# QwenLM/Qwen3-TTS

Hardware: NVIDIA B200
Metric: speech_tokens_per_s (higher is better)
Workload: dtype bf16

## Files before the change

qwen3-tts_b200/csrc/ar_sampler.cuh:

```cuda
#pragma once

namespace {

__device__ __forceinline__ unsigned int fkey(float f) {
  unsigned int u = __float_as_uint(f);
  return (u & 0x80000000u) ? ~u : (u | 0x80000000u);
}

__device__ __noinline__ float kth_largest(const float* sv, int V, int k, unsigned int* hist, int* sh) {
  unsigned int prefix = 0, mask = 0;
#pragma unroll 1
  for (int pass = 3; pass >= 0; --pass) {
    const int shift = pass * 8;
    if (threadIdx.x < 256) hist[threadIdx.x] = 0;
    cta_sync();
#pragma unroll 1
    for (int i = threadIdx.x; i < V; i += NTHREADS) {
      const unsigned int key = fkey(sv[i]);
      if ((key & mask) == prefix) atomicAdd(&hist[(key >> shift) & 255u], 1u);
    }
    cta_sync();
    unsigned int cnt = 0, incl = 0;
    if (threadIdx.x < 256) {
      cnt = hist[threadIdx.x];
      incl = cnt;
      const int ln = threadIdx.x & 31;
#pragma unroll
      for (int o = 1; o < 32; o <<= 1) {
        unsigned int n = __shfl_down_sync(0xffffffffu, incl, o);
        if (ln + o < 32) incl += n;
      }
      if (ln == 0) sh[threadIdx.x >> 5] = (int)incl;
    }
    cta_sync();
    if (threadIdx.x < 256) {
      unsigned int above = 0;
#pragma unroll 1
      for (int w = (threadIdx.x >> 5) + 1; w < 8; ++w) above += (unsigned int)sh[w];
      incl += above;
      const unsigned int excl = incl - cnt;
      if ((int)excl < k && k <= (int)incl) { sh[8] = threadIdx.x; sh[9] = k - (int)excl; }
    }
    cta_sync();
    prefix |= ((unsigned int)sh[8]) << shift;
    mask |= 255u << shift;
    k = sh[9];
    cta_sync();
  }
  const unsigned int u = (prefix & 0x80000000u) ? (prefix & 0x7fffffffu) : ~prefix;
  return __uint_as_float(u);
}

__device__ __noinline__ bool sample_fast(const float* sv, int V, int k, float u, float* scratch, float* red, int* ired, int* tok_out) {
  int* hist = reinterpret_cast<int*>(scratch);
  float* cand = scratch + 2048;
  int* kidx = reinterpret_cast<int*>(scratch + 2048 + 256);
  float* kp = scratch + 2048 + 256 + 384;
  int* sidx = reinterpret_cast<int*>(scratch + 2048 + 256 + 768);
  float* spp = scratch + 2048 + 256 + 1152;
  __shared__ int s_misc[8];
  const int tid = threadIdx.x, lane = tid & 31, wp = tid >> 5;
  float mx = -INFINITY;
#pragma unroll 1
  for (int i = tid; i < V; i += NTHREADS) mx = fmaxf(mx, sv[i]);
  mx = block_reduce(mx, red, 0);
#pragma unroll 1
  for (int i = tid; i < 2048; i += NTHREADS) hist[i] = 0;
  if (tid == 0) { s_misc[0] = -1; s_misc[2] = 0; s_misc[3] = 0; s_misc[4] = __float_as_int(-INFINITY); }
  cta_sync();
  const float lo = mx - 32.f;
#pragma unroll 1
  for (int i = tid; i < V; i += NTHREADS) {
    const float sc = sv[i];
    if (sc > -INFINITY) atomicAdd(&hist[min(2047, max(0, (int)((sc - lo) * 64.f)))], 1);
  }
  cta_sync();
  int hb[8], S = 0;
#pragma unroll
  for (int j = 0; j < 8; ++j) { hb[j] = hist[8 * tid + j]; S += hb[j]; }
  int incl = S;
#pragma unroll
  for (int o = 1; o < 32; o <<= 1) {
    const int n = __shfl_down_sync(0xffffffffu, incl, o);
    if (lane + o < 32) incl += n;
  }
  if (lane == 0) ired[wp] = incl;
  cta_sync();
  int above = incl - S;
#pragma unroll 1
  for (int w = wp + 1; w < NWARPS; ++w) above += ired[w];
  {
    int run = above;
#pragma unroll
    for (int j = 7; j >= 0; --j) {
      if (run < k && k <= run + hb[j]) { s_misc[0] = 8 * tid + j; s_misc[1] = k - run; }
      run += hb[j];
    }
  }
  cta_sync();
  const int tb = s_misc[0], kk = s_misc[1];
  if (tb < 0) return false;
#pragma unroll 1
  for (int i = tid; i < V; i += NTHREADS) {
    const float sc = sv[i];
    if (sc > -INFINITY && min(2047, max(0, (int)((sc - lo) * 64.f))) == tb) {
      const int p = atomicAdd(&s_misc[2], 1);
      if (p < 256) cand[p] = sc;
    }
  }
  cta_sync();
  const int nc = s_misc[2];
  if (nc > 256) return false;
  if (tid < nc) {
    const float v = cand[tid];
    int gt = 0, ge = 0;
#pragma unroll 1
    for (int j = 0; j < nc; ++j) { const float w = cand[j]; gt += w > v; ge += w >= v; }
    if (gt < kk && kk <= ge) s_misc[4] = __float_as_int(v);
  }
  cta_sync();
  const float thr = __int_as_float(s_misc[4]);
#pragma unroll 1
  for (int i = tid; i < V; i += NTHREADS) {
    const float sc = sv[i];
    if (sc > -INFINITY && sc >= thr) {
      const int p = atomicAdd(&s_misc[3], 1);
      if (p < 384) { kidx[p] = i; kp[p] = __expf(sc - mx); }
    }
  }
  cta_sync();
  const int m = s_misc[3];
  if (m > 384 || m == 0) return false;
#pragma unroll 1
  for (int e = tid; e < m; e += NTHREADS) {
    const int id = kidx[e];
    int r = 0;
#pragma unroll 1
    for (int j = 0; j < m; ++j) r += kidx[j] < id;
    sidx[r] = id;
    spp[r] = kp[e];
  }
  cta_sync();
  if (tid < 32) {
    const int per = (m + 31) >> 5;
    const int a = min(m, lane * per), bnd = min(m, a + per);
    float loc = 0.f;
#pragma unroll 1
    for (int j = a; j < bnd; ++j) loc += spp[j];
    float inc = loc;
#pragma unroll
    for (int o = 1; o < 32; o <<= 1) {
      const float n = __shfl_up_sync(0xffffffffu, inc, o);
      if (lane >= o) inc += n;
    }
    const float total = __shfl_sync(0xffffffffu, inc, 31);
    const float target = u * total;
    float run = inc - loc;
    int cnd = 0x7fffffff;
#pragma unroll 1
    for (int j = a; j < bnd; ++j) {
      run += spp[j];
      if (run > target && cnd == 0x7fffffff && spp[j] > 0.f) cnd = j;
    }
#pragma unroll
    for (int o = 16; o > 0; o >>= 1) cnd = min(cnd, __shfl_xor_sync(0xffffffffu, cnd, o));
    if (cnd == 0x7fffffff) {
      int last = -1;
#pragma unroll 1
      for (int j = a; j < bnd; ++j)
        if (spp[j] > 0.f) last = j;
#pragma unroll
      for (int o = 16; o > 0; o >>= 1) last = max(last, __shfl_xor_sync(0xffffffffu, last, o));
      cnd = max(last, 0);
    }
    if (lane == 0) s_misc[5] = sidx[cnd];
  }
  cta_sync();
  *tok_out = s_misc[5];
  return true;
}

__device__ __forceinline__ void sample_phase(const Phase& ph, const KParams& P, unsigned char* smem, int frame, bool in_prefill) {
  const int b = blockIdx.x;
  DevState* st = P.st;
  const int B = P.B;
  if (b >= B) return;
  if (in_prefill && !((P.admit_mask >> b) & 1u)) return;
  frame -= P.frame0[b];
  const int tid = threadIdx.x;
  const int group = ph.group;
  const bool talker = group == 0;
  const StackDev& S = talker ? P.talker : P.cp;
  const int V = S.vocab;
  const int H = P.talker.hidden;
  float* sv = reinterpret_cast<float*>(smem);
  float* pv = sv + MAXV;
  float* red = pv + MAXV;
  int* ired = reinterpret_cast<int*>(red + 32);
  unsigned int* hist = reinterpret_cast<unsigned int*>(ired + 32);
  const int fidx = talker ? (in_prefill ? 0 : frame + 1) : frame;
  const bool do_sample = talker ? P.sp.do_sample : P.sp.subtalker_dosample;
  const float temperature = talker ? P.sp.temperature : P.sp.subtalker_temperature;
  const int top_k = talker ? P.sp.top_k : P.sp.subtalker_top_k;
  const float top_p = talker ? P.sp.top_p : P.sp.subtalker_top_p;
  const float* lg = S.logits + (size_t)b * V;
  const int n_gen_b = talker ? ldcgi(&st->n_gen[b]) : 0;

  {
    float lreg[MAXV / NTHREADS];
#pragma unroll
    for (int r = 0; r < MAXV / NTHREADS; ++r) { const int i = tid + r * NTHREADS; if (i < V) lreg[r] = ldcgf(lg + i); }
#pragma unroll
    for (int r = 0; r < MAXV / NTHREADS; ++r) { const int i = tid + r * NTHREADS; if (i < V) sv[i] = lreg[r]; }
  }
  float* dbg = talker ? (P.dbg_tlogits ? P.dbg_tlogits + ((size_t)fidx * B + b) * V : nullptr)
                      : (P.dbg_clogits ? P.dbg_clogits + (((size_t)frame * (P.G - 1) + (group - 1)) * B + b) * V : nullptr);
  const float rp = P.sp.repetition_penalty;
  const float inv_t = (do_sample && temperature != 1.0f) ? temperature : 1.0f;
#pragma unroll 1
  for (int i = tid; i < V; i += NTHREADS) {
    float s = sv[i];
    if (dbg) dbg[i] = s;
    if (talker) {
      if (rp != 1.0f && __ldcg(P.seen + (size_t)b * V + i)) s = s < 0.f ? s * rp : s / rp;
      if (i == P.eos && (n_gen_b < P.sp.min_new_tokens || P.sp.suppress_eos)) s = -INFINITY;
      if (i >= V - 1024 && i != P.eos) s = -INFINITY;
    }
    if (inv_t != 1.0f) s = s / inv_t;
    sv[i] = s;
  }
  cta_sync();

  int tok;
  if (!do_sample) {
    float mx = -INFINITY;
#pragma unroll 1
    for (int i = tid; i < V; i += NTHREADS) mx = fmaxf(mx, sv[i]);
    mx = block_reduce(mx, red, 0);
    int idx = 0x7fffffff;
#pragma unroll 1
    for (int i = tid; i < V; i += NTHREADS)
      if (sv[i] == mx) idx = min(idx, i);
    tok = block_min_int(idx, ired);
  } else if (top_p >= 1.0f && top_k > 0 && top_k < V && top_k <= 128 &&
             sample_fast(sv, V, top_k, philox_uniform(P.sp.seed, P.row_key[b], (uint32_t)fidx, (uint32_t)group), pv, red, ired, &tok)) {
  } else {
    if (top_k > 0 && top_k < V) {
      const float thr = kth_largest(sv, V, top_k, hist, ired);
#pragma unroll 1
      for (int i = tid; i < V; i += NTHREADS)
        if (sv[i] < thr) sv[i] = -INFINITY;
      cta_sync();
    }
    float mx = -INFINITY;
#pragma unroll 1
    for (int i = tid; i < V; i += NTHREADS) mx = fmaxf(mx, sv[i]);
    mx = block_reduce(mx, red, 0);
    if (top_p < 1.0f) {
      float tot = 0.f;
#pragma unroll 1
      for (int i = tid; i < V; i += NTHREADS) { const float p = __expf(sv[i] - mx); pv[i] = p; tot += p; }
      tot = block_reduce(tot, red, 1);
      cta_sync();
      unsigned int rm_mask = 0;
      int slot = 0;
#pragma unroll 1
      for (int i = tid; i < V; i += NTHREADS, ++slot) {
        const float si = sv[i];
        bool rm = false;
        if (si != -INFINITY) {
          float cum = 0.f;
          bool is_top = true;
#pragma unroll 1
          for (int j = 0; j < V; ++j) {
            const float sj = sv[j];
            if (sj == -INFINITY) continue;
            if (sj < si || (sj == si && j <= i)) cum += pv[j];
            if (sj > si || (sj == si && j > i)) is_top = false;
          }
          rm = (cum / tot <= 1.0f - top_p) && !is_top;
        }
        if (rm) rm_mask |= 1u << slot;
      }
      cta_sync();
      slot = 0;
#pragma unroll 1
      for (int i = tid; i < V; i += NTHREADS, ++slot)
        if (rm_mask & (1u << slot)) sv[i] = -INFINITY;
      cta_sync();
    }
    const int E = (V + NTHREADS - 1) / NTHREADS;
    const int i0 = tid * E, i1 = min(V, i0 + E);
    float loc = 0.f;
#pragma unroll 1
    for (int i = i0; i < i1; ++i) { const float p = __expf(sv[i] - mx); pv[i] = p; loc += p; }
    float incl = loc;
    const int ln = tid & 31, wp = tid >> 5;
#pragma unroll
    for (int o = 1; o < 32; o <<= 1) {
      const float n = __shfl_up_sync(0xffffffffu, incl, o);
      if (ln >= o) incl += n;
    }
    cta_sync();
    if (ln == 31) red[wp] = incl;
    cta_sync();
    float base = 0.f, total = 0.f;
#pragma unroll 1
    for (int w = 0; w < NWARPS; ++w) { if (w < wp) base += red[w]; total += red[w]; }
    const float excl = base + incl - loc;
    const float u = philox_uniform(P.sp.seed, P.row_key[b], (uint32_t)fidx, (uint32_t)group);
    const float target = u * total;
    int cand = 0x7fffffff, lastpos = -1;
    float run = excl;
#pragma unroll 1
    for (int i = i0; i < i1; ++i) {
      run += pv[i];
      if (pv[i] > 0.f) { lastpos = i; if (run > target && cand == 0x7fffffff) cand = i; }
    }
    cand = block_min_int(cand, ired);
    if (cand == 0x7fffffff) cand = -block_min_int(-lastpos, ired);
    tok = cand;
  }
  if (P.forced && fidx < P.n_forced) {
    const int f = P.forced[((size_t)b * P.n_forced + fidx) * P.G + group];
    if (f >= 0) tok = f;
  }

  if (talker) {
    const int was_finished = ldcgi(&st->finished[b]);
    if (was_finished) tok = P.eos;
    cta_sync();
    if (tid == 0) {
      if (!was_finished) {
        if (tok == P.eos) { st->finished[b] = 1; st->n_valid[b] = fidx; }
        else { P.seen[(size_t)b * V + tok] = 1; }
        st->n_gen[b] = n_gen_b + 1;
      }
      st->c0[b] = tok;
      st->cur[b][0] = tok;
    }
    bf16* x1 = P.x_cp + ((size_t)B + b) * H;
    bf16* x0 = P.x_cp + (size_t)b * H;
    const bf16* e = P.emb_t + (size_t)tok * H;
    const bf16* ph_ = P.past_hidden + (size_t)b * H;
#pragma unroll 1
    for (int i = tid * 8; i < H; i += NTHREADS * 8) {
      *reinterpret_cast<uint4*>(x1 + i) = *reinterpret_cast<const uint4*>(e + i);
      *reinterpret_cast<uint4*>(x0 + i) = ldcg16(ph_ + i);
    }
  } else {
    const int j = group;
    if (tid == 0) {
      st->cur[b][j] = tok;
      if (P.codes_out && frame >= 0 && frame < P.codes_stride) {
        int* row = P.codes_out + ((size_t)b * P.codes_stride + frame) * P.G;
        row[j] = tok;
        if (j == 1) row[0] = ldcgi(&st->cur[b][0]);
      }
    }
    cta_sync();
    const int Vc = P.cp.vocab;
    if (j < P.G - 1) {
      const int Wn = P.cp_next_w;
      const bf16* e = P.cp_next + ((size_t)(j - 1) * Vc + tok) * Wn;
      bf16* x = P.cp_next_dst + (size_t)b * Wn;
#pragma unroll 1
      for (int i = tid * 8; i < Wn; i += NTHREADS * 8)
        *reinterpret_cast<uint4*>(x + i) = *reinterpret_cast<const uint4*>(e + i);
    } else {
      const bf16* txt = (frame < P.trailing_len[b])
                            ? P.trailing + ((size_t)b * P.trailing_stride + frame) * H
                            : P.tts_pad;
      int* codes = reinterpret_cast<int*>(hist);
      if (tid < P.G) codes[tid] = (tid == j) ? tok : ldcgi(&st->cur[b][tid]);
      cta_sync();
#pragma unroll 1
      for (int i = tid; i < H; i += NTHREADS) {
        float s = bf2f(P.emb_t[(size_t)codes[0] * H + i]);
#pragma unroll 4
        for (int g2 = 1; g2 < P.G; ++g2) s += bf2f(P.emb_cp[((size_t)(g2 - 1) * Vc + codes[g2]) * H + i]);
        P.talker.h[(size_t)b * H + i] = f2bf(rbf(s) + bf2f(txt[i]));
      }
    }
  }
}

}
```

Before: 2070.

## Fuse max into preprocessing and drop extra vocab pass in fast top-k sampler

The running max is now computed inside the penalty/temperature loop, which removes a separate pass over the vocabulary in both the greedy and sampling paths. The histogram is zeroed during preprocessing, so one barrier disappears. In the fast top-k sampler, the candidate-collection pass also gathers every token above the threshold bin, and candidates inside the threshold bin are selected directly by rank. This removes the final full-vocabulary threshold scan. The trade-off is extra shared scratch for candidate indices and a different ordering in kidx, which the later rank-sort handles.

```diff
diff --git a/qwen3-tts_b200/csrc/ar_sampler.cuh b/qwen3-tts_b200/csrc/ar_sampler.cuh
--- a/qwen3-tts_b200/csrc/ar_sampler.cuh
+++ b/qwen3-tts_b200/csrc/ar_sampler.cuh
@@ -51,23 +51,20 @@
   return __uint_as_float(u);
 }
 
-__device__ __noinline__ bool sample_fast(const float* sv, int V, int k, float u, float* scratch, float* red, int* ired, int* tok_out) {
+__device__ __noinline__ bool sample_fast(const float* sv, int V, int k, float u, float* scratch, float* red, int* ired, int* tok_out,
+                                         float mx_part) {
   int* hist = reinterpret_cast<int*>(scratch);
   float* cand = scratch + 2048;
-  int* kidx = reinterpret_cast<int*>(scratch + 2048 + 256);
-  float* kp = scratch + 2048 + 256 + 384;
-  int* sidx = reinterpret_cast<int*>(scratch + 2048 + 256 + 768);
-  float* spp = scratch + 2048 + 256 + 1152;
+  int* cidx = reinterpret_cast<int*>(scratch + 2048 + 256);
+  int* kidx = reinterpret_cast<int*>(scratch + 2048 + 512);
+  float* kp = scratch + 2048 + 512 + 384;
+  int* sidx = reinterpret_cast<int*>(scratch + 2048 + 512 + 768);
+  float* spp = scratch + 2048 + 512 + 1152;
+  static_assert(2048 + 512 + 1536 <= MAXV, "sampler scratch");
   __shared__ int s_misc[8];
   const int tid = threadIdx.x, lane = tid & 31, wp = tid >> 5;
-  float mx = -INFINITY;
-#pragma unroll 1
-  for (int i = tid; i < V; i += NTHREADS) mx = fmaxf(mx, sv[i]);
-  mx = block_reduce(mx, red, 0);
-#pragma unroll 1
-  for (int i = tid; i < 2048; i += NTHREADS) hist[i] = 0;
-  if (tid == 0) { s_misc[0] = -1; s_misc[2] = 0; s_misc[3] = 0; s_misc[4] = __float_as_int(-INFINITY); }
-  cta_sync();
+  if (tid == 0) { s_misc[0] = -1; s_misc[2] = 0; s_misc[3] = 0; }
+  const float mx = block_reduce(mx_part, red, 0);
   const float lo = mx - 32.f;
 #pragma unroll 1
   for (int i = tid; i < V; i += NTHREADS) {
@@ -103,9 +100,15 @@
 #pragma unroll 1
   for (int i = tid; i < V; i += NTHREADS) {
     const float sc = sv[i];
-    if (sc > -INFINITY && min(2047, max(0, (int)((sc - lo) * 64.f))) == tb) {
-      const int p = atomicAdd(&s_misc[2], 1);
-      if (p < 256) cand[p] = sc;
+    if (sc > -INFINITY) {
+      const int bin = min(2047, max(0, (int)((sc - lo) * 64.f)));
+      if (bin == tb) {
+        const int p = atomicAdd(&s_misc[2], 1);
+        if (p < 256) { cand[p] = sc; cidx[p] = i; }
+      } else if (bin > tb) {
+        const int p = atomicAdd(&s_misc[3], 1);
+        if (p < 384) { kidx[p] = i; kp[p] = __expf(sc - mx); }
+      }
     }
   }
   cta_sync();
@@ -113,19 +116,12 @@
   if (nc > 256) return false;
   if (tid < nc) {
     const float v = cand[tid];
-    int gt = 0, ge = 0;
-#pragma unroll 1
-    for (int j = 0; j < nc; ++j) { const float w = cand[j]; gt += w > v; ge += w >= v; }
-    if (gt < kk && kk <= ge) s_misc[4] = __float_as_int(v);
-  }
-  cta_sync();
-  const float thr = __int_as_float(s_misc[4]);
-#pragma unroll 1
-  for (int i = tid; i < V; i += NTHREADS) {
-    const float sc = sv[i];
-    if (sc > -INFINITY && sc >= thr) {
+    int gt = 0;
+#pragma unroll 1
+    for (int j = 0; j < nc; ++j) gt += cand[j] > v;
+    if (gt < kk) {
       const int p = atomicAdd(&s_misc[3], 1);
-      if (p < 384) { kidx[p] = i; kp[p] = __expf(sc - mx); }
+      if (p < 384) { kidx[p] = cidx[tid]; kp[p] = __expf(v - mx); }
     }
   }
   cta_sync();
@@ -217,6 +213,13 @@
                       : (P.dbg_clogits ? P.dbg_clogits + (((size_t)frame * (P.G - 1) + (group - 1)) * B + b) * V : nullptr);
   const float rp = P.sp.repetition_penalty;
   const float inv_t = (do_sample && temperature != 1.0f) ? temperature : 1.0f;
+  const bool fast = do_sample && top_p >= 1.0f && top_k > 0 && top_k < V && top_k <= 128;
+  if (fast) {
+    int* hz = reinterpret_cast<int*>(pv);
+#pragma unroll 1
+    for (int i = tid; i < 2048; i += NTHREADS) hz[i] = 0;
+  }
+  float mx_part = -INFINITY;
 #pragma unroll 1
   for (int i = tid; i < V; i += NTHREADS) {
     float s = sv[i];
@@ -228,22 +231,20 @@
     }
     if (inv_t != 1.0f) s = s / inv_t;
     sv[i] = s;
+    mx_part = fmaxf(mx_part, s);
   }
   cta_sync();
 
   int tok;
   if (!do_sample) {
-    float mx = -INFINITY;
-#pragma unroll 1
-    for (int i = tid; i < V; i += NTHREADS) mx = fmaxf(mx, sv[i]);
-    mx = block_reduce(mx, red, 0);
+    const float mx = block_reduce(mx_part, red, 0);
     int idx = 0x7fffffff;
 #pragma unroll 1
     for (int i = tid; i < V; i += NTHREADS)
       if (sv[i] == mx) idx = min(idx, i);
     tok = block_min_int(idx, ired);
-  } else if (top_p >= 1.0f && top_k > 0 && top_k < V && top_k <= 128 &&
-             sample_fast(sv, V, top_k, philox_uniform(P.sp.seed, P.row_key[b], (uint32_t)fidx, (uint32_t)group), pv, red, ired, &tok)) {
+  } else if (fast && sample_fast(sv, V, top_k, philox_uniform(P.sp.seed, P.row_key[b], (uint32_t)fidx, (uint32_t)group), pv, red, ired,
+                                 &tok, mx_part)) {
   } else {
     if (top_k > 0 && top_k < V) {
       const float thr = kth_largest(sv, V, top_k, hist, ired);
```

Result: no change. 2076 (median of 6 runs) (+0.3%).
